# fabrii4/AutoEncoder-FFT

Measured on AMD Instinct MI355X. Metric: frames/s fwd+bwd (FFT mode, 512x512, 4 layers), higher is better.
Workload: dtype f32; 1 GPU; cfg3-P2: 512x512x3 frames, 4 pairs 3->8->16->32->64, 5x5, pool 2/layer, FFT mode, fwd + 1 loop-body iteration per pair (operator form); every step produces reconstructions, batch-mean gradients, updated weights and the per-pair post-update MSE partial sums -- the sums themselves are formed by the next step's gradient launch (no per-step MSE read-back inside the timed loop); frames_per_gpu=32, global_batch=32, parallelism=dp1

## Files before the change

autoencoder-fft_amd/csrc/fft_kernels.hip:

```cpp
#include "internal.h"
#include "device_util.h"
#include "fft_common.h"
#include "score_device.h"
#include <hip/hip_ext.h>
#include <math.h>
#include <map>
#include <mutex>
#include <vector>

namespace aefft {

__device__ float2 g_tw[TW_N];

hipError_t upload_twiddles(hipStream_t st)
{
    static std::vector<float2> host;
    if (host.empty()) {
        host.resize(TW_N);
        for (int k = 0; k < TW_N; ++k) {
            double a = -2.0 * M_PI * (double)k / (double)TW_N;
            host[k] = make_float2((float)cos(a), (float)sin(a));
        }
    }
    hipError_t e = hipMemcpyToSymbolAsync(HIP_SYMBOL(g_tw), host.data(), sizeof(float2) * TW_N, 0, hipMemcpyHostToDevice, st);
    if (e != hipSuccess) return e;
    return hipStreamSynchronize(st);
}

const float2* twiddle_table()
{
    void* p = nullptr;
    if (hipGetSymbolAddress(&p, HIP_SYMBOL(g_tw)) != hipSuccess) return nullptr;
    return static_cast<const float2*>(p);
}

bool fft_size_supported(int n) { return n >= 8 && n <= 2048 && (n & (n - 1)) == 0; }

template <int DIR> __device__ __forceinline__ float2 twid(int idx)
{
    float2 w = g_tw[idx];
    if (DIR > 0) w.y = -w.y;
    return w;
}

template <int N> __device__ __forceinline__ void pass_sync()
{
    if constexpr (N / 8 <= 64) __builtin_amdgcn_wave_barrier();
    else __syncthreads();
}

template <int N, int R, int S, int DIR>
__device__ __forceinline__ void fft_pass(float2* s, int t, float2 w1)
{
    constexpr int T = N / 8;
    constexpr int E = 8 / R;
    constexpr int n = N / S;
    float2 a[8];
#pragma unroll
    for (int v = 0; v < E; ++v) {
        const int ib = t + T * v;
#pragma unroll
        for (int tt = 0; tt < R; ++tt) a[v * R + tt] = s[pad_idx(ib + tt * (N / R))];
    }
    pass_sync<N>();
#pragma unroll
    for (int v = 0; v < E; ++v) {
        const int ib = t + T * v;
        const int p = ib / S, q = ib % S;
        Dft<R, DIR>::run(&a[v * R]);
        if constexpr (n > R) {
            static_assert(R == 8 && E == 1, "twiddled passes are radix 8");
            const float2 w2 = cmul(w1, w1), w3 = cmul(w2, w1), w4 = cmul(w2, w2);
            const float2 w5 = cmul(w4, w1), w6 = cmul(w3, w3), w7 = cmul(w4, w3);
            a[1] = cmul(a[1], w1); a[2] = cmul(a[2], w2); a[3] = cmul(a[3], w3); a[4] = cmul(a[4], w4);
            a[5] = cmul(a[5], w5); a[6] = cmul(a[6], w6); a[7] = cmul(a[7], w7);
        }
#pragma unroll
        for (int u = 0; u < R; ++u) s[pad_idx(q + S * (R * p + u))] = a[v * R + u];
    }
    if constexpr (S * R == N) __syncthreads();
    else pass_sync<N>();
}

template <int N, int DIR> struct FftTw {
    float2 w[3];
    __device__ __forceinline__ void load(int t)
    {
        constexpr int S[3] = {1, 8, 64};
#pragma unroll
        for (int i = 0; i < 3; ++i) {
            w[i] = make_float2(1.f, 0.f);
            if (N / S[i] > 8) {
                float2 v = g_tw[((t / S[i]) * S[i]) * (TW_N / N)];
                if (DIR > 0) v.y = -v.y;
                w[i] = v;
            }
        }
    }
};

template <int N, int S, int I, int DIR> struct Passes {
    static __device__ __forceinline__ void run(float2* s, int t, const FftTw<N, DIR>& tw)
    {
        constexpr int n = N / S;
        constexpr int R = n >= 8 ? 8 : n;
        fft_pass<N, R, S, DIR>(s, t, tw.w[I < 3 ? I : 2]);
        Passes<N, S * R, I + 1, DIR>::run(s, t, tw);
    }
};
template <int N, int I, int DIR> struct Passes<N, N, I, DIR> {
    static __device__ __forceinline__ void run(float2*, int, const FftTw<N, DIR>&) {}
};

template <int N, int DIR> __device__ __forceinline__ void fft_lds(float2* s, int t, const FftTw<N, DIR>& tw) { Passes<N, 1, 0, DIR>::run(s, t, tw); }

template <int N> struct RowCfg {
    static constexpr int T = N / 8;
    static constexpr int NT = T > 256 ? T : 256;
    static constexpr int G = NT / T;
    static constexpr int PL = pad_len(N);
};

template <int N, bool U8>
__global__ __launch_bounds__(RowCfg<N>::NT) void r2c_rows_kernel(const void* __restrict__ in_v, float2* __restrict__ mid,
                                                                   long npairs, int Wc)
{
    using Cfg = RowCfg<N>;
    constexpr int T = Cfg::T, NT = Cfg::NT, G = Cfg::G, PL = Cfg::PL;
    extern __shared__ float2 s[];
    const int tid = threadIdx.x;
    const int g = tid / T, t = tid % T;
    const long pair0 = (long)blockIdx.x * G;
    FftTw<N, -1> tws;
    tws.load(t);

    constexpr int NPOS = G * (N / 4) / NT;
    static_assert((G * (N / 4)) % NT == 0, "tile must be a whole number of positions per thread");
    const int live = npairs - pair0 < G ? (int)(npairs - pair0) : G;
    float4 va[NPOS], vb[NPOS];
    if constexpr (U8) {
        const unsigned* src = reinterpret_cast<const unsigned*>(static_cast<const unsigned char*>(in_v) + pair0 * 2 * N);
        unsigned wa[NPOS], wb[NPOS];
#pragma unroll
        for (int q = 0; q < NPOS; ++q) {
            const int pos = tid + q * NT;
            const int gg = pos / (N / 4), c4 = pos % (N / 4);
            const int idx = gg < live ? gg * (2 * N / 4) + c4 : c4;
            wa[q] = __builtin_nontemporal_load(&src[idx]);
            wb[q] = __builtin_nontemporal_load(&src[idx + N / 4]);
        }
#pragma unroll
        for (int q = 0; q < NPOS; ++q) {
            va[q] = make_float4((float)(wa[q] & 255u), (float)((wa[q] >> 8) & 255u), (float)((wa[q] >> 16) & 255u), (float)(wa[q] >> 24));
            vb[q] = make_float4((float)(wb[q] & 255u), (float)((wb[q] >> 8) & 255u), (float)((wb[q] >> 16) & 255u), (float)(wb[q] >> 24));
        }
    } else {
        const float4* src = reinterpret_cast<const float4*>(static_cast<const float*>(in_v) + pair0 * 2 * N);
#pragma unroll
        for (int q = 0; q < NPOS; ++q) {
            const int pos = tid + q * NT;
            const int gg = pos / (N / 4), c4 = pos % (N / 4);
            const int idx = gg < live ? gg * (2 * N / 4) + c4 : c4;
            va[q] = ld_stream(&src[idx]);
            vb[q] = ld_stream(&src[idx + N / 4]);
        }
    }
#pragma unroll
    for (int q = 0; q < NPOS; ++q) {
        const int pos = tid + q * NT;
        const int gg = pos / (N / 4), c4 = pos % (N / 4);
        if (gg < live) {
            float2* z = s + gg * PL + pad_idx(4 * c4);
            z[0] = make_float2(va[q].x, vb[q].x); z[1] = make_float2(va[q].y, vb[q].y);
            z[2] = make_float2(va[q].z, vb[q].z); z[3] = make_float2(va[q].w, vb[q].w);
        }
    }
    __syncthreads();
    fft_lds<N, -1>(s + g * PL, t, tws);

    const int half = Wc / 2, hs = 31 - __builtin_clz(half);
    float2* const obase = mid + pair0 * 2 * Wc;
    for (int it = tid; it < G * half; it += NT) {
        const int gg = it >> hs, k = (it & (half - 1)) * 2;
        if (gg >= live) continue;
        const float2* z = s + gg * PL;
        const float2 zk1 = z[pad_idx(k + 1)], zn1 = z[pad_idx(N - k - 1)];
        float2 a0, b0;
        if (k == 0) {
            const float2 z0 = z[pad_idx(0)], zh = z[pad_idx(N / 2)];
            a0 = make_float2(z0.x, zh.x); b0 = make_float2(z0.y, zh.y);
        } else {
            const float2 zk = z[pad_idx(k)], zn = z[pad_idx(N - k)];
            a0 = make_float2(0.5f * (zk.x + zn.x), 0.5f * (zk.y - zn.y)); b0 = make_float2(0.5f * (zk.y + zn.y), -0.5f * (zk.x - zn.x));
        }
        const float2 a1 = make_float2(0.5f * (zk1.x + zn1.x), 0.5f * (zk1.y - zn1.y)), b1 = make_float2(0.5f * (zk1.y + zn1.y), -0.5f * (zk1.x - zn1.x));
        float2* dst = obase + (gg * 2 * Wc + k);
        *reinterpret_cast<float4*>(dst) = make_float4(a0.x, a0.y, a1.x, a1.y);
        *reinterpret_cast<float4*>(dst + Wc) = make_float4(b0.x, b0.y, b1.x, b1.y);
    }
}

template <int N, bool SPARSE, bool U8 = false, int SCORE = 0>
__global__ __launch_bounds__(RowCfg<N>::NT) void c2r_rows_kernel(const float2* __restrict__ mid, void* __restrict__ out_v,
                                                                   long npairs, int Wc, float scale, const typename ScoreParam<SCORE>::type sc)
{
    using Cfg = RowCfg<N>;
    constexpr int T = Cfg::T, NT = Cfg::NT, G = Cfg::G, PL = Cfg::PL;
    static_assert(!(U8 && SCORE), "the scoring epilogue has no 8-bit reconstruction");
    extern __shared__ float2 s[];
    const int tid = threadIdx.x;
    const int g = tid / T, t = tid % T;
    FftTw<N, +1> tws;
    tws.load(t);
    const long pair0 = (long)blockIdx.x * G;
    constexpr int NQ = G * (N / 4) / NT;
    using Tr = ScoreTraits<SCORE>;
    [[maybe_unused]] ScoreRef<4, Tr::F32> ref[NQ];
    [[maybe_unused]] auto load_frames = [&](int lv) {
        if constexpr (SCORE != 0) {
#pragma unroll
            for (int q = 0; q < NQ; ++q) {
                const int idx = tid + q * NT;
                const int gg = idx / (N / 4), n4 = idx % (N / 4);
                const int off = (gg < lv ? gg * (2 * N / 4) : 0) + n4;
                ref[q].load(score_rows<Tr::F32>(sc.frames, pair0 * 2 * N), off, off + N / 4);
            }
        }
    };
    if constexpr (SPARSE) {
        static_assert(N >= 128, "sparse head: three radix-8 passes or more");
        const int live = npairs - pair0 < G ? (int)(npairs - pair0) : G;
        const float2* const ibase = mid + pair0 * 2 * Wc;
        const bool lo = t < Wc, hi = t > T - Wc;
        const int k = lo ? t : (hi ? T - t : 0);
        const bool ok = g < live && (lo || hi);
        const int off = ok ? g * 2 * Wc + k : 0;
        float2 A = ibase[off], B = ibase[off + Wc];
        load_frames(live);
        if (!ok) { A = make_float2(0.f, 0.f); B = A; }
        const float2 zz = make_float2(0.f, 0.f);
        const float2 a0 = lo ? (t == 0 ? make_float2(A.x, B.x) : make_float2(A.x - B.y, A.y + B.x)) : zz;
        const float2 a4 = t == 0 ? make_float2(A.y, B.y) : zz;
        const float2 a7 = hi ? make_float2(A.x + B.y, -A.y + B.x) : zz;
        const float c = 0.70710678118654752440f;
        const float2 e = cadd(a0, a4), o = csub(a0, a4);
        const float2 r1 = make_float2(c * (a7.x + a7.y), c * (a7.y - a7.x));
        const float2 r2 = make_float2(a7.y, -a7.x);
        const float2 r3 = make_float2(c * (a7.y - a7.x), -c * (a7.x + a7.y));
        float2 x[8] = {cadd(e, a7), cadd(o, r1), cadd(e, r2), cadd(o, r3), csub(e, a7), csub(o, r1), csub(e, r2), csub(o, r3)};
        const float2 w1 = tws.w[0];
        const float2 w2 = cmul(w1, w1), w3 = cmul(w2, w1), w4 = cmul(w2, w2);
        const float2 w5 = cmul(w4, w1), w6 = cmul(w3, w3), w7 = cmul(w4, w3);
        x[1] = cmul(x[1], w1); x[2] = cmul(x[2], w2); x[3] = cmul(x[3], w3); x[4] = cmul(x[4], w4);
        x[5] = cmul(x[5], w5); x[6] = cmul(x[6], w6); x[7] = cmul(x[7], w7);
        float2* z = s + g * PL;
#pragma unroll
        for (int u = 0; u < 8; ++u) z[pad_idx(8 * t + u)] = x[u];
        pass_sync<N>();
        Passes<N, 8, 1, +1>::run(z, t, tws);
    } else {
    constexpr int NIT = G * (N / 4) / NT;
    static_assert((G * (N / 4)) % NT == 0, "tile must be a whole number of items per thread");
    float4 av[NIT], bv[NIT];
    const int live = npairs - pair0 < G ? (int)(npairs - pair0) : G;
    const float2* const ibase = mid + pair0 * 2 * Wc;
#pragma unroll
    for (int q = 0; q < NIT; ++q) {
        const int it = tid + q * NT;
        const int gg = it / (N / 4), k = (it % (N / 4)) * 2;
        const bool ok = gg < live && k < Wc;
        const int off = ok ? gg * 2 * Wc + k : 0;
        av[q] = ld_stream(reinterpret_cast<const float4*>(ibase + off));
        bv[q] = ld_stream(reinterpret_cast<const float4*>(ibase + off + Wc));
        if (!ok) { av[q] = make_float4(0.f, 0.f, 0.f, 0.f); bv[q] = av[q]; }
    }
    load_frames(live);
#pragma unroll
    for (int q = 0; q < NIT; ++q) {
        const int it = tid + q * NT;
        const int gg = it / (N / 4), k = (it % (N / 4)) * 2;
        if (gg >= live) continue;
        float2* z = s + gg * PL;
        const float4 a = av[q], b = bv[q];
        if (k == 0) {
            z[pad_idx(0)] = make_float2(a.x, b.x);
            z[pad_idx(N / 2)] = make_float2(a.y, b.y);
        } else {
            z[pad_idx(k)] = make_float2(a.x - b.y, a.y + b.x);
            z[pad_idx(N - k)] = make_float2(a.x + b.y, -a.y + b.x);
        }
        z[pad_idx(k + 1)] = make_float2(a.z - b.w, a.w + b.z);
        z[pad_idx(N - k - 1)] = make_float2(a.z + b.w, -a.w + b.z);
    }
    __syncthreads();
    fft_lds<N, +1>(s + g * PL, t, tws);
    }

    const int live = npairs - pair0 < G ? (int)(npairs - pair0) : G;
    if constexpr (SCORE != 0) {
        float* const orow = static_cast<float*>(out_v) + pair0 * 2 * N;
        const bool store = out_v != nullptr;
        ScoreAcc<Tr::NS> acc[NQ];
#pragma unroll
        for (int q = 0; q < NQ; ++q) {
            const int idx = tid + q * NT;
            const int gg = idx / (N / 4), n = (idx % (N / 4)) * 4;
            acc[q].clear();
            if (gg < live)
                score_position(s + gg * PL + pad_idx(n), scale, ref[q], score_pivot(sc), store, orow + (gg * 2) * N + n, orow + (gg * 2 + 1) * N + n, acc[q]);
        }
        if constexpr (Tr::STRIP) {
            const int lw = sc.lt - 2, ns = N >> sc.lt;
            const long ms = npairs * ns;
#pragma unroll
            for (int q = 0; q < NQ; ++q) {
                const int idx = tid + q * NT;
                const int gg = idx / (N / 4), n4 = idx % (N / 4);
                score_strip_reduce<4>(acc[q], lw, (n4 & ((1 << lw) - 1)) == 0 && gg < live, sc.part + (pair0 + gg) * ns + (n4 >> lw), ms);
            }
            return;
        }
        constexpr int LPP = N / 4 < NT ? N / 4 : NT;
        constexpr int NR = N / 4 <= NT ? NQ : 1;
        if constexpr (N / 4 > NT) acc[0].m[0] += acc[1].m[0];
        if constexpr (LPP <= 64) {
#pragma unroll
            for (int q = 0; q < NR; ++q) {
                const float v = score_seg_sum<LPP>(acc[q].m[0]);
                const int gg = (tid + q * NT) / (N / 4);
                if (tid % LPP == 0 && gg < live) sc.part[pair0 + gg] = v;
            }
        } else {
            __shared__ float red[NR][NT / 64];
#pragma unroll
            for (int q = 0; q < NR; ++q) {
                const float v = score_seg_sum<64>(acc[q].m[0]);
                if ((tid & 63) == 0) red[q][tid >> 6] = v;
            }
            __syncthreads();
#pragma unroll
            for (int q = 0; q < NR; ++q) {
                const int gg = N / 4 > NT ? 0 : (tid + q * NT) / (N / 4);
                if (tid % LPP == 0 && gg < live) {
                    float v = red[q][tid >> 6];
#pragma unroll
                    for (int w = 1; w < LPP / 64; ++w) v += red[q][(tid >> 6) + w];
                    sc.part[pair0 + gg] = v;
                }
            }
        }
        return;
    }
    if constexpr (U8) {
        unsigned* const orow = reinterpret_cast<unsigned*>(static_cast<unsigned char*>(out_v) + pair0 * 2 * N);
#pragma unroll
        for (int q = 0; q < NQ; ++q) {
            const int idx = tid + q * NT;
            const int gg = idx / (N / 4), n4 = idx % (N / 4);
            if (gg < live) {
                const float2* z = s + gg * PL + pad_idx(4 * n4);
                const float2 z0 = z[0], z1 = z[1], z2 = z[2], z3 = z[3];
                const unsigned wa = px_u8(z0.x * scale) | px_u8(z1.x * scale) << 8 | px_u8(z2.x * scale) << 16 | px_u8(z3.x * scale) << 24;
                const unsigned wb = px_u8(z0.y * scale) | px_u8(z1.y * scale) << 8 | px_u8(z2.y * scale) << 16 | px_u8(z3.y * scale) << 24;
                __builtin_nontemporal_store(wa, &orow[(gg * 2) * (N / 4) + n4]);
                __builtin_nontemporal_store(wb, &orow[(gg * 2 + 1) * (N / 4) + n4]);
            }
        }
        return;
    }
    float* const orow = static_cast<float*>(out_v) + pair0 * 2 * N;
#pragma unroll
    for (int q = 0; q < NQ; ++q) {
        const int idx = tid + q * NT;
        const int gg = idx / (N / 4), n = (idx % (N / 4)) * 4;
        if (gg < live) {
            const float2* z = s + gg * PL + pad_idx(n);
            const float2 z0 = z[0], z1 = z[1], z2 = z[2], z3 = z[3];
            st_stream(reinterpret_cast<float4*>(orow + (gg * 2) * N + n), make_float4(z0.x * scale, z1.x * scale, z2.x * scale, z3.x * scale));
            st_stream(reinterpret_cast<float4*>(orow + (gg * 2 + 1) * N + n), make_float4(z0.y * scale, z1.y * scale, z2.y * scale, z3.y * scale));
        }
    }
}

template <int N, int CW>
__global__ __launch_bounds__(CW* N / 8) void fwd_cols_kernel(const float2* __restrict__ mid, float2* __restrict__ out,
                                                              int Wc, int Nxs)
{
    constexpr int T = N / 8, NT = CW * T, PL = pad_len(N);
    extern __shared__ float2 s[];
    const int tid = threadIdx.x;
    FftTw<N, -1> tws;
    tws.load(tid % T);
    const long plane = blockIdx.x;
    const int c0 = blockIdx.y * CW;

    const float2* src = mid + plane * N * (long)Wc + c0;
    constexpr int NLD = N * (CW / 2) / NT;
    float4 val[NLD];
#pragma unroll
    for (int k = 0; k < NLD; ++k) {
        const int it = tid + k * NT;
        const float4* ptr = reinterpret_cast<const float4*>(src + ((it / (CW / 2)) * Wc + 2 * (it % (CW / 2))));
        if constexpr (CW * sizeof(float2) >= 128) val[k] = ld_stream(ptr);
        else val[k] = *ptr;
    }
#pragma unroll
    for (int k = 0; k < NLD; ++k) {
        const int it = tid + k * NT;
        const int r = it / (CW / 2), c2 = it % (CW / 2);
        s[(2 * c2) * PL + pad_idx(r)] = make_float2(val[k].x, val[k].y);
        s[(2 * c2 + 1) * PL + pad_idx(r)] = make_float2(val[k].z, val[k].w);
    }
    __syncthreads();
    fft_lds<N, -1>(s + (tid / T) * PL, tid % T, tws);

    const int Nyrs = Wc + 1;
    float2* dst = out + plane * Nxs * (long)Nyrs;
    for (int it = tid; it < Nxs * CW; it += NT) {
        const int i = it / CW, c = it % CW;
        const int si = crop_row(i, N, Nxs);
        const float2 z = s[c * PL + pad_idx(si)];
        const int col = c0 + c;
        if (col == 0) {
            const float2 zn = s[pad_idx((N - si) % N)];
            dst[i * Nyrs] = make_float2(0.5f * (z.x + zn.x), 0.5f * (z.y - zn.y));
            dst[i * Nyrs + Wc] = make_float2(0.5f * (z.y + zn.y), -0.5f * (z.x - zn.x));
        } else {
            dst[i * Nyrs + col] = z;
        }
    }
}

template <int N, int CW>
__global__ __launch_bounds__(CW* N / 8) void inv_cols_kernel(const float2* __restrict__ in, float2* __restrict__ mid,
                                                              int Wc, int Nxi, const OpIn op)
{
    constexpr int T = N / 8, NT = CW * T, PL = pad_len(N);
    extern __shared__ float2 s[];
    const int tid = threadIdx.x;
    FftTw<N, +1> tws;
    tws.load(tid % T);
    const long plane = blockIdx.x;
    const int c0 = blockIdx.y * CW;
    const int Nyri = Wc + 1;
    const float2* src = in + plane * Nxi * (long)Nyri;
    auto ld = [&](long t) { return op.A ? opin_load(op, plane, (int)t, Nxi, 2 * Wc) : src[t]; };

    float2* dcs = s + CW * PL;
    float2* nys = dcs + Nxi;
    if (Nxi < N) {
        for (int it = tid; it < CW * PL; it += NT) s[it] = make_float2(0.f, 0.f);
        __syncthreads();
    }
    constexpr int NLD = 8;
    float2 v[NLD], w[NLD];
    const int nsrc = Nxi * CW;
#pragma unroll
    for (int k = 0; k < NLD; ++k) {
        if (k * NT < nsrc) {
            const int it = min(tid + k * NT, nsrc - 1);
            const int sr = it / CW, c = it % CW;
            v[k] = ld((long)sr * Nyri + c0 + c);
            w[k] = (c0 + c == 0) ? ld((long)sr * Nyri + Wc) : make_float2(0.f, 0.f);
        }
    }
#pragma unroll
    for (int k = 0; k < NLD; ++k) {
        const int it = tid + k * NT;
        if (it < nsrc) {
            const int sr = it / CW, c = it % CW;
            if (c0 + c == 0) { dcs[sr] = v[k]; nys[sr] = w[k]; }
            else {
                const int r = Nxi == N ? sr : (sr < Nxi / 2 ? sr : (sr == Nxi / 2 ? N / 2 : sr + N - Nxi));
                s[c * PL + pad_idx(r)] = v[k];
            }
        }
    }
    if (c0 == 0) {
        __syncthreads();
        for (int r = tid; r < N; r += NT) {
            const int sr = padsrc_row(r, N, Nxi), sm = padsrc_row((N - r) % N, N, Nxi);
            const float2 zz = make_float2(0.f, 0.f);
            const float2 d0 = sr >= 0 ? dcs[sr] : zz, n0 = sr >= 0 ? nys[sr] : zz, d1 = sm >= 0 ? dcs[sm] : zz, n1 = sm >= 0 ? nys[sm] : zz;
            const float2 dc = make_float2(0.5f * (d0.x + d1.x), 0.5f * (d0.y - d1.y));
            const float2 ny = make_float2(0.5f * (n0.x + n1.x), 0.5f * (n0.y - n1.y));
            s[pad_idx(r)] = make_float2(dc.x - ny.y, dc.y + ny.x);
        }
    }
    __syncthreads();
    fft_lds<N, +1>(s + (tid / T) * PL, tid % T, tws);

    float2* dst = mid + plane * N * (long)Wc + c0;
    for (int it = tid; it < N * (CW / 2); it += NT) {
        const int r = it / (CW / 2), c2 = it % (CW / 2);
        const float2 a = s[(2 * c2) * PL + pad_idx(r)], b = s[(2 * c2 + 1) * PL + pad_idx(r)];
        *reinterpret_cast<float4*>(dst + (long)r * Wc + 2 * c2) = make_float4(a.x, a.y, b.x, b.y);
    }
}

template <int M> struct BluCfg {
    static constexpr int T = M / 8;
    static constexpr int NT = T > 256 ? T : 256;
    static constexpr int G = NT / T;
    static constexpr int PL = pad_len(M);
};

template <int M, int MODE>
__global__ __launch_bounds__(BluCfg<M>::NT) void bluestein_rows_kernel(const void* __restrict__ in_, void* __restrict__ out_, const float2* __restrict__ tab,
                                                                        long nrows, int n, float scale)
{
    using Cfg = BluCfg<M>;
    constexpr int T = Cfg::T, NT = Cfg::NT, G = Cfg::G, PL = Cfg::PL;
    extern __shared__ float2 s[];
    const int tid = threadIdx.x, g = tid / T, t = tid % T;
    const long row = (long)blockIdx.x * G + g;
    const bool live = row < nrows;
    FftTw<M, -1> twf;
    FftTw<M, +1> twi;
    twf.load(t); twi.load(t);
    float2* z = s + g * PL;
    const float2* const bhat = tab;
    const float2* const w = tab + M;
    const int nh = n / 2 + 1;
    for (int j = t; j < M; j += T) {
        float2 v = make_float2(0.f, 0.f);
        if (live && j < n) {
            if (MODE == 0) v = reinterpret_cast<const float2*>(in_)[row * n + j];
            else if (MODE == 1) v = make_float2(reinterpret_cast<const float*>(in_)[row * n + j], 0.f);
            else {
                const float2* X = reinterpret_cast<const float2*>(in_) + row * nh;
                if (j < nh) { v = X[j]; if (j == 0 || 2 * j == n) v.y = 0.f; }
                else { v = X[n - j]; v.y = -v.y; }
            }
            v = cmul(v, w[j]);
        }
        z[pad_idx(j)] = v;
    }
    __syncthreads();
    fft_lds<M, -1>(z, t, twf);
    for (int j = t; j < M; j += T) z[pad_idx(j)] = cmul(z[pad_idx(j)], bhat[j]);
    __syncthreads();
    fft_lds<M, +1>(z, t, twi);
    if (!live) return;
    const float sc = scale / (float)M;
    const int nout = MODE == 1 ? nh : n;
    for (int k = t; k < nout; k += T) {
        float2 v = cmul(z[pad_idx(k)], w[k]);
        if (MODE == 2) reinterpret_cast<float*>(out_)[row * n + k] = v.x * sc;
        else reinterpret_cast<float2*>(out_)[row * nout + k] = make_float2(v.x * sc, v.y * sc);
    }
}

__global__ __launch_bounds__(256) void transpose_c_kernel(const float2* __restrict__ in, float2* __restrict__ out, int R, int C)
{
    __shared__ float2 tile[32][33];
    const long plane = blockIdx.z;
    const int r0 = blockIdx.y * 32, c0 = blockIdx.x * 32;
    const int tx = threadIdx.x % 32, ty = threadIdx.x / 32;
    for (int k = ty; k < 32; k += 8) if (r0 + k < R && c0 + tx < C) tile[k][tx] = in[(plane * R + r0 + k) * C + c0 + tx];
    __syncthreads();
    for (int k = ty; k < 32; k += 8) if (c0 + k < C && r0 + tx < R) out[(plane * C + c0 + k) * R + r0 + tx] = tile[tx][k];
}

size_t fft_mid_elems(long planes, int Nx, int Wc) { return (size_t)planes * Nx * Wc; }

template <typename K> static hipError_t allow_lds(K kernel, size_t bytes)
{
    if (bytes <= 64 * 1024) return hipSuccess;
    return hipFuncSetAttribute(reinterpret_cast<const void*>(kernel), hipFuncAttributeMaxDynamicSharedMemorySize, (int)bytes);
}

template <int N> static hipError_t run_r2c_rows(const void* in, float2* mid, long npairs, int Wc, hipStream_t st, bool in_u8)
{
    using Cfg = RowCfg<N>;
    const size_t lds = sizeof(float2) * (Cfg::G * Cfg::PL);
    hipError_t e = in_u8 ? allow_lds(r2c_rows_kernel<N, true>, lds) : allow_lds(r2c_rows_kernel<N, false>, lds);
    if (e != hipSuccess) return e;
    const long blocks = (npairs + Cfg::G - 1) / Cfg::G;
    if (in_u8) r2c_rows_kernel<N, true><<<dim3((unsigned)blocks), dim3(Cfg::NT), lds, st>>>(in, mid, npairs, Wc);
    else r2c_rows_kernel<N, false><<<dim3((unsigned)blocks), dim3(Cfg::NT), lds, st>>>(in, mid, npairs, Wc);
    return hipGetLastError();
}
template <int N, bool SPARSE, bool U8, int SCORE = 0>
static hipError_t run_c2r_rows_as(const float2* mid, void* out, long npairs, int Wc, float scale, hipStream_t st, const typename ScoreParam<SCORE>::type sc = {})
{
    using Cfg = RowCfg<N>;
    const size_t lds = sizeof(float2) * (Cfg::G * Cfg::PL);
    const long blocks = (npairs + Cfg::G - 1) / Cfg::G;
    hipError_t e = allow_lds(c2r_rows_kernel<N, SPARSE, U8, SCORE>, lds);
    if (e != hipSuccess) return e;
    c2r_rows_kernel<N, SPARSE, U8, SCORE><<<dim3((unsigned)blocks), dim3(Cfg::NT), lds, st>>>(mid, out, npairs, Wc, scale, sc);
    return hipGetLastError();
}
template <int N, bool SPARSE> static hipError_t run_c2r_rows_sp(const float2* mid, void* out, long npairs, int Wc, float scale, hipStream_t st, bool out_u8, const ScoreArg* score)
{
    if (score)
        return score_dispatch(*score, N, out_u8, [&](auto S, const auto& dev) {
            return run_c2r_rows_as<N, SPARSE, false, decltype(S)::value>(mid, out, npairs, Wc, scale, st, dev);
        });
    return out_u8 ? run_c2r_rows_as<N, SPARSE, true>(mid, out, npairs, Wc, scale, st) : run_c2r_rows_as<N, SPARSE, false>(mid, out, npairs, Wc, scale, st);
}
template <int N> static hipError_t run_c2r_rows(const float2* mid, void* out, long npairs, int Wc, float scale, hipStream_t st, bool out_u8, const ScoreArg* score)
{
    if constexpr (N >= 128) {
        if (Wc <= N / 16)
            return run_c2r_rows_sp<N, true>(mid, out, npairs, Wc, scale, st, out_u8, score);
    }
    return run_c2r_rows_sp<N, false>(mid, out, npairs, Wc, scale, st, out_u8, score);
}
template <int N, int CW> static hipError_t run_fwd_cols(const float2* mid, float2* out, long planes, int Wc, int Nxs, hipStream_t st, hipEvent_t done)
{
    const size_t lds = sizeof(float2) * (CW * pad_len(N));
    hipError_t e = allow_lds(fwd_cols_kernel<N, CW>, lds);
    if (e != hipSuccess) return e;
    if (done) hipExtLaunchKernelGGL((fwd_cols_kernel<N, CW>), dim3((unsigned)planes, Wc / CW), dim3(CW * N / 8), lds, st, nullptr, done, 0, mid, out, Wc, Nxs);
    else fwd_cols_kernel<N, CW><<<dim3((unsigned)planes, Wc / CW), dim3(CW * N / 8), lds, st>>>(mid, out, Wc, Nxs);
    return hipGetLastError();
}
static OpIn g_opin_none{};
template <int N, int CW> static hipError_t run_inv_cols(const float2* in, float2* mid, long planes, int Wc, int Nxi, hipStream_t st, const OpIn& op = g_opin_none)
{
    const size_t lds = sizeof(float2) * (CW * pad_len(N) + 2 * Nxi);
    hipError_t e = allow_lds(inv_cols_kernel<N, CW>, lds);
    if (e != hipSuccess) return e;
    inv_cols_kernel<N, CW><<<dim3((unsigned)planes, Wc / CW), dim3(CW * N / 8), lds, st>>>(in, mid, Wc, Nxi, op);
    return hipGetLastError();
}

template <int N, bool FWD> static hipError_t cols_dispatch(const float2* a, float2* b, long planes, int Wc, int Nother, hipStream_t st, const OpIn& op = g_opin_none, hipEvent_t done = nullptr)
{
    constexpr int CWMAX = (8192 / N) < 16 ? (8192 / N) : 16;
    int cw = CWMAX;
    while (cw > Wc) cw >>= 1;
    if (!FWD) while (cw > 4 && planes * (Wc / cw) < 256) cw >>= 1;
#define AEFFT_CW_CASE(C)                                                                                   \
    if constexpr (C <= CWMAX) {                                                                             \
        if (cw == C) return FWD ? run_fwd_cols<N, C>(a, b, planes, Wc, Nother, st, done) : run_inv_cols<N, C>(a, b, planes, Wc, Nother, st, op); \
    }
    AEFFT_CW_CASE(16) AEFFT_CW_CASE(8) AEFFT_CW_CASE(4)
#undef AEFFT_CW_CASE
    return hipErrorInvalidValue;
}

#define AEFFT_N_SWITCH(n, CALL)                       \
    switch (n) {                                      \
    case 8: { constexpr int NN = 8; CALL; }           \
    case 16: { constexpr int NN = 16; CALL; }         \
    case 32: { constexpr int NN = 32; CALL; }         \
    case 64: { constexpr int NN = 64; CALL; }         \
    case 128: { constexpr int NN = 128; CALL; }       \
    case 256: { constexpr int NN = 256; CALL; }       \
    case 512: { constexpr int NN = 512; CALL; }       \
    case 1024: { constexpr int NN = 1024; CALL; }     \
    case 2048: { constexpr int NN = 2048; CALL; }     \
    default: e = hipErrorInvalidValue;                \
    }

bool fft_size_supported_any(int n) { return fft_size_supported(n) || (n >= 8 && n <= 1024 && (n & 1) == 0); }
static int blu_m(int n) { int m = 16; while (m < 2 * n - 1) m *= 2; return m; }
struct BluKey { int dev, n, dir; bool operator<(const BluKey& o) const { return dev != o.dev ? dev < o.dev : (n != o.n ? n < o.n : dir < o.dir); } };
#define AEFFT_M_SWITCH(m, CALL)                      \
    switch (m) {                                      \
    case 16: { constexpr int MM = 16; CALL; }         \
    case 32: { constexpr int MM = 32; CALL; }         \
    case 64: { constexpr int MM = 64; CALL; }         \
    case 128: { constexpr int MM = 128; CALL; }       \
    case 256: { constexpr int MM = 256; CALL; }       \
    case 512: { constexpr int MM = 512; CALL; }       \
    case 1024: { constexpr int MM = 1024; CALL; }     \
    case 2048: { constexpr int MM = 2048; CALL; }     \
    default: e = hipErrorInvalidValue;                \
    }
static std::mutex g_blu_mu;
static std::vector<float2> blu_host_table(int n, int dir)
{
    const int M = blu_m(n);
    std::vector<double> wr(n), wi(n), cr(M), ci(M);
    for (int j = 0; j < n; ++j) {
        const long q = ((long)j * j) % (2L * n);
        wr[j] = cos(M_PI * (double)q / n); wi[j] = dir * sin(M_PI * (double)q / n);
    }
    for (int m = 0; m < M; ++m) { cr[m] = cos(2.0 * M_PI * m / M); ci[m] = -sin(2.0 * M_PI * m / M); }
    std::vector<float2> t(M + n);
    for (int k = 0; k < M; ++k) {
        double ar = 0.0, ai = 0.0;
        for (int j = 0; j < M; ++j) {
            const int jj = j < n ? j : (M - j < n ? M - j : -1);
            if (jj < 0) continue;
            const double br = wr[jj], bi = -wi[jj];
            const int m = (int)(((long)j * k) % M);
            ar += br * cr[m] - bi * ci[m]; ai += br * ci[m] + bi * cr[m];
        }
        t[k] = make_float2((float)ar, (float)ai);
    }
    for (int j = 0; j < n; ++j) t[M + j] = make_float2((float)wr[j], (float)wi[j]);
    return t;
}
static hipError_t blu_table(int n, int dir, const float2** out)
{
    static std::map<BluKey, float2*> cache;
    int dev = 0;
    hipError_t e = hipGetDevice(&dev);
    if (e != hipSuccess) return e;
    const BluKey key{dev, n, dir};
    std::lock_guard<std::mutex> lock(g_blu_mu);
    auto it = cache.find(key);
    if (it == cache.end()) {
        const std::vector<float2> host = blu_host_table(n, dir);
        float2* p = nullptr;
        e = hipMalloc(&p, sizeof(float2) * host.size());
        if (e != hipSuccess) return e;
        e = hipMemcpy(p, host.data(), sizeof(float2) * host.size(), hipMemcpyHostToDevice);
        if (e != hipSuccess) { (void)hipFree(p); return e; }
        it = cache.emplace(key, p).first;
    }
    *out = it->second;
    return hipSuccess;
}
template <int M, int MODE> static hipError_t run_blu_rows(const void* in, void* out, const float2* tab, long nrows, int n, float scale, hipStream_t st)
{
    using Cfg = BluCfg<M>;
    const size_t lds = sizeof(float2) * (size_t)Cfg::G * Cfg::PL;
    hipError_t e = allow_lds(bluestein_rows_kernel<M, MODE>, lds);
    if (e != hipSuccess) return e;
    const long blocks = (nrows + Cfg::G - 1) / Cfg::G;
    if (blocks >= (1L << 31)) return hipErrorInvalidValue;
    bluestein_rows_kernel<M, MODE><<<dim3((unsigned)blocks), dim3(Cfg::NT), lds, st>>>(in, out, tab, nrows, n, scale);
    return hipGetLastError();
}
static hipError_t blu_rows(int mode, const void* in, void* out, long nrows, int n, int dir, float scale, hipStream_t st)
{
    const float2* tab = nullptr;
    hipError_t e = blu_table(n, dir, &tab);
    if (e != hipSuccess) return e;
    const int M = blu_m(n);
    if (mode == 0) { AEFFT_M_SWITCH(M, e = (run_blu_rows<MM, 0>(in, out, tab, nrows, n, scale, st)); break) }
    else if (mode == 1) { AEFFT_M_SWITCH(M, e = (run_blu_rows<MM, 1>(in, out, tab, nrows, n, scale, st)); break) }
    else { AEFFT_M_SWITCH(M, e = (run_blu_rows<MM, 2>(in, out, tab, nrows, n, scale, st)); break) }
    return e;
}
static hipError_t transpose_c(const float2* in, float2* out, long planes, int R, int C, hipStream_t st)
{
    constexpr long ZMAX = 65535;
    for (long p0 = 0; p0 < planes; p0 += ZMAX) {
        const long np = planes - p0 < ZMAX ? planes - p0 : ZMAX;
        const long off = p0 * R * (long)C;
        transpose_c_kernel<<<dim3((C + 31) / 32, (R + 31) / 32, (unsigned)np), 256, 0, st>>>(in + off, out + off, R, C);
        hipError_t e = hipGetLastError();
        if (e != hipSuccess) return e;
    }
    return hipSuccess;
}
size_t fft_any_ws_elems(long planes, int Nx, int Ny) { return (size_t)planes * Nx * (Ny / 2 + 1); }
hipError_t launch_r2c_any(const float* in, float2* out, float2* w1, float2* w2, long planes, int Nx, int Ny, hipStream_t st)
{
    if (!fft_size_supported_any(Nx) || !fft_size_supported_any(Ny) || Nx > 1024 || Ny > 1024) return hipErrorInvalidValue;
    if (planes <= 0) return hipSuccess;
    const int Nyr = Ny / 2 + 1;
    hipError_t e = blu_rows(1, in, w1, planes * Nx, Ny, -1, 1.f, st);
    if (e == hipSuccess) e = transpose_c(w1, w2, planes, Nx, Nyr, st);
    if (e == hipSuccess) e = blu_rows(0, w2, w1, planes * Nyr, Nx, -1, 1.f, st);
    if (e == hipSuccess) e = transpose_c(w1, out, planes, Nyr, Nx, st);
    return e;
}
hipError_t launch_c2r_any(const float2* in, float* out, float2* w1, float2* w2, long planes, int Nx, int Ny, float scale, hipStream_t st)
{
    if (!fft_size_supported_any(Nx) || !fft_size_supported_any(Ny) || Nx > 1024 || Ny > 1024) return hipErrorInvalidValue;
    if (planes <= 0) return hipSuccess;
    const int Nyr = Ny / 2 + 1;
    hipError_t e = transpose_c(in, w1, planes, Nx, Nyr, st);
    if (e == hipSuccess) e = blu_rows(0, w1, w2, planes * Nyr, Nx, +1, 1.f, st);
    if (e == hipSuccess) e = transpose_c(w2, w1, planes, Nyr, Nx, st);
    if (e == hipSuccess) e = blu_rows(2, w1, out, planes * Nx, Ny, +1, scale, st);
    return e;
}

static bool rows_pow2(int Ny, int Wc) { return fft_size_supported(Ny) && Wc >= 4 && (Wc & (Wc - 1)) == 0; }
static bool cols_pow2(int Nx, int Wc) { return fft_size_supported(Nx) && Wc >= 4 && ((Wc & (Wc - 1)) == 0 || Wc % 16 == 0); }
static bool axis_ok(int n) { return fft_size_supported(n) || fft_size_mixed(n); }

hipError_t launch_r2c(const void* in, float2* out, float2* mid, long planes, int Nx, int Ny, int Nxs, int Nys, hipStream_t st, hipEvent_t done, bool in_u8)
{
    if (!fft_size_supported(Nx) || !fft_size_supported(Ny) || Nxs > Nx || Nys > Ny || Nys < 8 || Nxs < 2 || (Nys & (Nys - 1)) || (Nxs & 1)) {
        if (!axis_ok(Nx) || !axis_ok(Ny) || Nxs > Nx || Nys > Ny || Nxs < 2 || Nys < 2 || (Nxs & 1) || (Nys & 1)) return hipErrorInvalidValue;
        if (planes <= 0) return hipSuccess;
        const int Wc = Nys / 2;
        const long npairs = planes * Nx / 2;
        hipError_t e = hipSuccess;
        if (in) {
            if (rows_pow2(Ny, Wc)) { AEFFT_N_SWITCH(Ny, e = run_r2c_rows<NN>(in, mid, npairs, Wc, st, in_u8); break) }
            else e = launch_mix_r2c_rows(in, mid, npairs, Ny, Wc, st, in_u8);
            if (e != hipSuccess) return e;
        }
        if (out) {
            if (cols_pow2(Nx, Wc)) { AEFFT_N_SWITCH(Nx, e = (cols_dispatch<NN, true>(mid, out, planes, Wc, Nxs, st, g_opin_none, done)); break) }
            else e = launch_mix_fwd_cols(mid, out, planes, Nx, Wc, Nxs, st, done);
        }
        return e;
    }
    if (planes <= 0) return hipSuccess;
    const int Wc = Nys / 2;
    const long npairs = planes * Nx / 2;
    hipError_t e = hipSuccess;
    if (in) {
        AEFFT_N_SWITCH(Ny, e = run_r2c_rows<NN>(in, mid, npairs, Wc, st, in_u8); break)
        if (e != hipSuccess) return e;
    }
    if (out) {
        AEFFT_N_SWITCH(Nx, e = (cols_dispatch<NN, true>(mid, out, planes, Wc, Nxs, st, g_opin_none, done)); break)
    }
    return e;
}

hipError_t launch_c2r(const float2* in, void* out, float2* mid, long planes, int Nxi, int Nyi, int Nx, int Ny, float scale, hipStream_t st, const OpIn* opin,
                      bool out_u8, const ScoreArg* score)
{
    const OpIn op = opin ? *opin : g_opin_none;
    if ((Nxi == Nx) != (Nyi == Ny)) return hipErrorInvalidValue;
    if (!fft_size_supported(Nx) || !fft_size_supported(Ny) || Nxi > Nx || Nyi > Ny || Nyi < 8 || Nxi < 2 || (Nyi & 1) || (Nxi & 1)) {
        if (!axis_ok(Nx) || !axis_ok(Ny) || Nxi > Nx || Nyi > Ny || Nxi < 2 || Nyi < 2 || (Nxi & 1) || (Nyi & 1)) return hipErrorInvalidValue;
        if (planes <= 0) return hipSuccess;
        const int Wc = Nyi / 2;
        const long npairs = planes * Nx / 2;
        hipError_t e = hipSuccess;
        if (in || op.A) {
            if (cols_pow2(Nx, Wc)) { AEFFT_N_SWITCH(Nx, e = (cols_dispatch<NN, false>(in, mid, planes, Wc, Nxi, st, op)); break) }
            else e = launch_mix_inv_cols(in, mid, planes, Nx, Wc, Nxi, st, op.A ? &op : nullptr);
            if (e != hipSuccess) return e;
        }
        if (out || score) {
            if (rows_pow2(Ny, Wc)) { AEFFT_N_SWITCH(Ny, e = run_c2r_rows<NN>(mid, out, npairs, Wc, scale, st, out_u8, score); break) }
            else e = launch_mix_c2r_rows(mid, out, npairs, Ny, Wc, scale, st, out_u8, score);
        }
        return e;
    }
    if (planes <= 0) return hipSuccess;
    const int Wc = Nyi / 2;
    const long npairs = planes * Nx / 2;
    hipError_t e = hipSuccess;
    if (in || op.A) {
        AEFFT_N_SWITCH(Nx, e = (cols_dispatch<NN, false>(in, mid, planes, Wc, Nxi, st, op)); break)
        if (e != hipSuccess) return e;
    }
    if (out || score) {
        AEFFT_N_SWITCH(Ny, e = run_c2r_rows<NN>(mid, out, npairs, Wc, scale, st, out_u8, score); break)
    }
    return e;
}

}
```

Baseline: 233,100 frames/s.

## Load forward FFT rows straight into registers and write column-major intermediate

The forward real-to-complex row kernel now loads each thread's eight strided samples directly into registers and runs the first radix-8 pass from registers. This skips the initial shared-memory staging and one barrier. The row kernel also writes its intermediate spectrum in a transposed, column-contiguous layout, so the column FFT kernel can read its inputs straight into registers with strided loads instead of a shared-memory transpose. Blocks get larger (more rows per block) with tuned LDS pitches to avoid bank conflicts. The price is more scattered global writes in the row kernel, and other consumers of the intermediate buffer must match the new layout.

```diff
diff --git a/autoencoder-fft_amd/csrc/fft_kernels.hip b/autoencoder-fft_amd/csrc/fft_kernels.hip
--- a/autoencoder-fft_amd/csrc/fft_kernels.hip
+++ b/autoencoder-fft_amd/csrc/fft_kernels.hip
@@ -82,6 +82,22 @@
     else pass_sync<N>();
 }
 
+template <int N, int DIR>
+__device__ __forceinline__ void fft_pass_first_regs(float2* s, int t, float2 (&a)[8], float2 w1)
+{
+    Dft<8, DIR>::run(a);
+    if constexpr (N > 8) {
+        const float2 w2 = cmul(w1, w1), w3 = cmul(w2, w1), w4 = cmul(w2, w2);
+        const float2 w5 = cmul(w4, w1), w6 = cmul(w3, w3), w7 = cmul(w4, w3);
+        a[1] = cmul(a[1], w1); a[2] = cmul(a[2], w2); a[3] = cmul(a[3], w3); a[4] = cmul(a[4], w4);
+        a[5] = cmul(a[5], w5); a[6] = cmul(a[6], w6); a[7] = cmul(a[7], w7);
+    }
+#pragma unroll
+    for (int u = 0; u < 8; ++u) s[pad_idx(8 * t + u)] = a[u];
+    if constexpr (N == 8) __syncthreads();
+    else pass_sync<N>();
+}
+
 template <int N, int DIR> struct FftTw {
     float2 w[3];
     __device__ __forceinline__ void load(int t)
@@ -113,6 +129,11 @@
 };
 
 template <int N, int DIR> __device__ __forceinline__ void fft_lds(float2* s, int t, const FftTw<N, DIR>& tw) { Passes<N, 1, 0, DIR>::run(s, t, tw); }
+template <int N, int DIR> __device__ __forceinline__ void fft_lds_regs(float2* s, int t, float2 (&a)[8], const FftTw<N, DIR>& tw)
+{
+    fft_pass_first_regs<N, DIR>(s, t, a, tw.w[0]);
+    Passes<N, 8, 1, DIR>::run(s, t, tw);
+}
 
 template <int N> struct RowCfg {
     static constexpr int T = N / 8;
@@ -121,24 +142,36 @@
     static constexpr int PL = pad_len(N);
 };
 
+template <int N> struct FwdRowCfg {
+    static constexpr int T = N / 8;
+    static constexpr int WANT = 8 * T > 256 ? 8 * T : 256;
+    static constexpr int NT = WANT > 1024 ? 1024 : WANT;
+    static constexpr int G = NT / T;
+};
+template <int N> struct FwdRowPitch {
+    static constexpr int G = FwdRowCfg<N>::G;
+    static constexpr int MINP = pad_idx(N - 1) + 1;
+    static constexpr int PL = G >= 32 ? (pad_len(N) | 1) : (G == 4 ? MINP + (8 + 32 - MINP % 32) % 32 : pad_len(N));
+    static_assert(PL >= MINP, "pitch holds a padded transform");
+};
+
 template <int N, bool U8>
-__global__ __launch_bounds__(RowCfg<N>::NT) void r2c_rows_kernel(const void* __restrict__ in_v, float2* __restrict__ mid,
-                                                                   long npairs, int Wc)
-{
-    using Cfg = RowCfg<N>;
-    constexpr int T = Cfg::T, NT = Cfg::NT, G = Cfg::G, PL = Cfg::PL;
+__global__ __launch_bounds__(FwdRowCfg<N>::NT) void r2c_rows_kernel(const void* __restrict__ in_v, float2* __restrict__ mid,
+                                                                   long npairs, int Wc, int lxh)
+{
+    using Cfg = FwdRowCfg<N>;
+    constexpr int T = Cfg::T, NT = Cfg::NT, G = Cfg::G, PL = FwdRowPitch<N>::PL;
     extern __shared__ float2 s[];
     const int tid = threadIdx.x;
     const int g = tid / T, t = tid % T;
     const long pair0 = (long)blockIdx.x * G;
     FftTw<N, -1> tws;
     tws.load(t);
-
-    constexpr int NPOS = G * (N / 4) / NT;
-    static_assert((G * (N / 4)) % NT == 0, "tile must be a whole number of positions per thread");
     const int live = npairs - pair0 < G ? (int)(npairs - pair0) : G;
-    float4 va[NPOS], vb[NPOS];
+
     if constexpr (U8) {
+        constexpr int NPOS = G * (N / 4) / NT;
+        static_assert((G * (N / 4)) % NT == 0, "tile must be a whole number of positions per thread");
         const unsigned* src = reinterpret_cast<const unsigned*>(static_cast<const unsigned char*>(in_v) + pair0 * 2 * N);
         unsigned wa[NPOS], wb[NPOS];
 #pragma unroll
@@ -151,37 +184,37 @@
         }
 #pragma unroll
         for (int q = 0; q < NPOS; ++q) {
-            va[q] = make_float4((float)(wa[q] & 255u), (float)((wa[q] >> 8) & 255u), (float)((wa[q] >> 16) & 255u), (float)(wa[q] >> 24));
-            vb[q] = make_float4((float)(wb[q] & 255u), (float)((wb[q] >> 8) & 255u), (float)((wb[q] >> 16) & 255u), (float)(wb[q] >> 24));
-        }
-    } else {
-        const float4* src = reinterpret_cast<const float4*>(static_cast<const float*>(in_v) + pair0 * 2 * N);
-#pragma unroll
-        for (int q = 0; q < NPOS; ++q) {
             const int pos = tid + q * NT;
             const int gg = pos / (N / 4), c4 = pos % (N / 4);
-            const int idx = gg < live ? gg * (2 * N / 4) + c4 : c4;
-            va[q] = ld_stream(&src[idx]);
-            vb[q] = ld_stream(&src[idx + N / 4]);
-        }
-    }
-#pragma unroll
-    for (int q = 0; q < NPOS; ++q) {
-        const int pos = tid + q * NT;
-        const int gg = pos / (N / 4), c4 = pos % (N / 4);
-        if (gg < live) {
-            float2* z = s + gg * PL + pad_idx(4 * c4);
-            z[0] = make_float2(va[q].x, vb[q].x); z[1] = make_float2(va[q].y, vb[q].y);
-            z[2] = make_float2(va[q].z, vb[q].z); z[3] = make_float2(va[q].w, vb[q].w);
-        }
-    }
-    __syncthreads();
-    fft_lds<N, -1>(s + g * PL, t, tws);
-
-    const int half = Wc / 2, hs = 31 - __builtin_clz(half);
-    float2* const obase = mid + pair0 * 2 * Wc;
+            if (gg < live) {
+                float2* z = s + gg * PL + pad_idx(4 * c4);
+                z[0] = make_float2((float)(wa[q] & 255u), (float)(wb[q] & 255u));
+                z[1] = make_float2((float)((wa[q] >> 8) & 255u), (float)((wb[q] >> 8) & 255u));
+                z[2] = make_float2((float)((wa[q] >> 16) & 255u), (float)((wb[q] >> 16) & 255u));
+                z[3] = make_float2((float)(wa[q] >> 24), (float)(wb[q] >> 24));
+            }
+        }
+        __syncthreads();
+        fft_lds<N, -1>(s + g * PL, t, tws);
+    } else {
+        const float* src = static_cast<const float*>(in_v) + (pair0 + (g < live ? g : 0)) * 2 * N + t;
+        float xa[8], xb[8];
+#pragma unroll
+        for (int tt = 0; tt < 8; ++tt) xa[tt] = __builtin_nontemporal_load(&src[tt * T]);
+#pragma unroll
+        for (int tt = 0; tt < 8; ++tt) xb[tt] = __builtin_nontemporal_load(&src[N + tt * T]);
+        float2 a[8];
+#pragma unroll
+        for (int tt = 0; tt < 8; ++tt) a[tt] = make_float2(xa[tt], xb[tt]);
+        fft_lds_regs<N, -1>(s + g * PL, t, a, tws);
+    }
+
+    constexpr int LG = __builtin_ctz(G);
+    const int half = Wc / 2, hx = (1 << lxh) - 1;
+    const int rp0 = (int)(pair0 & hx);
+    float2* const obase = mid + (((pair0 >> lxh) * Wc) << (lxh + 1));
     for (int it = tid; it < G * half; it += NT) {
-        const int gg = it >> hs, k = (it & (half - 1)) * 2;
+        const int gg = it & (G - 1), k = (it >> LG) * 2;
         if (gg >= live) continue;
         const float2* z = s + gg * PL;
         const float2 zk1 = z[pad_idx(k + 1)], zn1 = z[pad_idx(N - k - 1)];
@@ -194,9 +227,10 @@
             a0 = make_float2(0.5f * (zk.x + zn.x), 0.5f * (zk.y - zn.y)); b0 = make_float2(0.5f * (zk.y + zn.y), -0.5f * (zk.x - zn.x));
         }
         const float2 a1 = make_float2(0.5f * (zk1.x + zn1.x), 0.5f * (zk1.y - zn1.y)), b1 = make_float2(0.5f * (zk1.y + zn1.y), -0.5f * (zk1.x - zn1.x));
-        float2* dst = obase + (gg * 2 * Wc + k);
-        *reinterpret_cast<float4*>(dst) = make_float4(a0.x, a0.y, a1.x, a1.y);
-        *reinterpret_cast<float4*>(dst + Wc) = make_float4(b0.x, b0.y, b1.x, b1.y);
+        const int q = rp0 + gg;
+        float2* dst = obase + ((((q >> lxh) * Wc + k) << (lxh + 1)) + 2 * (q & hx));
+        *reinterpret_cast<float4*>(dst) = make_float4(a0.x, a0.y, b0.x, b0.y);
+        *reinterpret_cast<float4*>(dst + (2 << lxh)) = make_float4(a1.x, a1.y, b1.x, b1.y);
     }
 }
 
@@ -389,30 +423,17 @@
     constexpr int T = N / 8, NT = CW * T, PL = pad_len(N);
     extern __shared__ float2 s[];
     const int tid = threadIdx.x;
+    const int tc = tid / T, t = tid % T;
     FftTw<N, -1> tws;
-    tws.load(tid % T);
+    tws.load(t);
     const long plane = blockIdx.x;
     const int c0 = blockIdx.y * CW;
 
-    const float2* src = mid + plane * N * (long)Wc + c0;
-    constexpr int NLD = N * (CW / 2) / NT;
-    float4 val[NLD];
-#pragma unroll
-    for (int k = 0; k < NLD; ++k) {
-        const int it = tid + k * NT;
-        const float4* ptr = reinterpret_cast<const float4*>(src + ((it / (CW / 2)) * Wc + 2 * (it % (CW / 2))));
-        if constexpr (CW * sizeof(float2) >= 128) val[k] = ld_stream(ptr);
-        else val[k] = *ptr;
-    }
-#pragma unroll
-    for (int k = 0; k < NLD; ++k) {
-        const int it = tid + k * NT;
-        const int r = it / (CW / 2), c2 = it % (CW / 2);
-        s[(2 * c2) * PL + pad_idx(r)] = make_float2(val[k].x, val[k].y);
-        s[(2 * c2 + 1) * PL + pad_idx(r)] = make_float2(val[k].z, val[k].w);
-    }
-    __syncthreads();
-    fft_lds<N, -1>(s + (tid / T) * PL, tid % T, tws);
+    const float2* src = mid + (plane * Wc + c0) * N + (tc * N + t);
+    float2 a[8];
+#pragma unroll
+    for (int tt = 0; tt < 8; ++tt) a[tt] = ld_stream(&src[tt * T]);
+    fft_lds_regs<N, -1>(s + tc * PL, t, a, tws);
 
     const int Nyrs = Wc + 1;
     float2* dst = out + plane * Nxs * (long)Nyrs;
@@ -570,15 +591,17 @@
     return hipFuncSetAttribute(reinterpret_cast<const void*>(kernel), hipFuncAttributeMaxDynamicSharedMemorySize, (int)bytes);
 }
 
-template <int N> static hipError_t run_r2c_rows(const void* in, float2* mid, long npairs, int Wc, hipStream_t st, bool in_u8)
-{
-    using Cfg = RowCfg<N>;
-    const size_t lds = sizeof(float2) * (Cfg::G * Cfg::PL);
+template <int N> static hipError_t run_r2c_rows(const void* in, float2* mid, long npairs, int Nx, int Wc, hipStream_t st, bool in_u8)
+{
+    using Cfg = FwdRowCfg<N>;
+    if (Nx < 2 || (Nx & (Nx - 1))) return hipErrorInvalidValue;
+    const int lxh = __builtin_ctz((unsigned)Nx) - 1;
+    const size_t lds = sizeof(float2) * (Cfg::G * FwdRowPitch<N>::PL);
     hipError_t e = in_u8 ? allow_lds(r2c_rows_kernel<N, true>, lds) : allow_lds(r2c_rows_kernel<N, false>, lds);
     if (e != hipSuccess) return e;
     const long blocks = (npairs + Cfg::G - 1) / Cfg::G;
-    if (in_u8) r2c_rows_kernel<N, true><<<dim3((unsigned)blocks), dim3(Cfg::NT), lds, st>>>(in, mid, npairs, Wc);
-    else r2c_rows_kernel<N, false><<<dim3((unsigned)blocks), dim3(Cfg::NT), lds, st>>>(in, mid, npairs, Wc);
+    if (in_u8) r2c_rows_kernel<N, true><<<dim3((unsigned)blocks), dim3(Cfg::NT), lds, st>>>(in, mid, npairs, Wc, lxh);
+    else r2c_rows_kernel<N, false><<<dim3((unsigned)blocks), dim3(Cfg::NT), lds, st>>>(in, mid, npairs, Wc, lxh);
     return hipGetLastError();
 }
 template <int N, bool SPARSE, bool U8, int SCORE = 0>
@@ -787,13 +810,14 @@
         const int Wc = Nys / 2;
         const long npairs = planes * Nx / 2;
         hipError_t e = hipSuccess;
+        const bool p2 = rows_pow2(Ny, Wc) && cols_pow2(Nx, Wc);
         if (in) {
-            if (rows_pow2(Ny, Wc)) { AEFFT_N_SWITCH(Ny, e = run_r2c_rows<NN>(in, mid, npairs, Wc, st, in_u8); break) }
+            if (p2) { AEFFT_N_SWITCH(Ny, e = run_r2c_rows<NN>(in, mid, npairs, Nx, Wc, st, in_u8); break) }
             else e = launch_mix_r2c_rows(in, mid, npairs, Ny, Wc, st, in_u8);
             if (e != hipSuccess) return e;
         }
         if (out) {
-            if (cols_pow2(Nx, Wc)) { AEFFT_N_SWITCH(Nx, e = (cols_dispatch<NN, true>(mid, out, planes, Wc, Nxs, st, g_opin_none, done)); break) }
+            if (p2) { AEFFT_N_SWITCH(Nx, e = (cols_dispatch<NN, true>(mid, out, planes, Wc, Nxs, st, g_opin_none, done)); break) }
             else e = launch_mix_fwd_cols(mid, out, planes, Nx, Wc, Nxs, st, done);
         }
         return e;
@@ -803,7 +827,7 @@
     const long npairs = planes * Nx / 2;
     hipError_t e = hipSuccess;
     if (in) {
-        AEFFT_N_SWITCH(Ny, e = run_r2c_rows<NN>(in, mid, npairs, Wc, st, in_u8); break)
+        AEFFT_N_SWITCH(Ny, e = run_r2c_rows<NN>(in, mid, npairs, Nx, Wc, st, in_u8); break)
         if (e != hipSuccess) return e;
     }
     if (out) {
```

Result: no change. 235,400 frames/s, median of 5 (+1.0%).
